# ajyoon/rocoder

Measured on AMD Instinct MI355X. Metric: output Msamples/s, 16384-win f=8 stereo (x CPU-realtime in config), higher is better.
Workload: dtype f32

## Files before the change

rocoder_amd/csrc/rc_hop16k.hip:

```cpp
#include "rc_dit.hpp"

namespace rc {
namespace {

constexpr int f1_idx(int n) { return n + (n >> 5); }
constexpr int HOP2_XBUF = 8192 + 256 + 32;
constexpr int HOP2_LDS_FLOAT2 = HOP2_XBUF + 8 + 32 + 256 + 256 + 16 + 24 + 1024;
constexpr int F3_W[13] = {1, 2, 4, 8, 16, 32, 64, 131, 259, 520, 1038, 2079, 4156};
constexpr int f3_idx(int n) {
    int r = 0;
    for (int i = 0; i < 13; ++i) r += ((n >> i) & 1) * F3_W[i];
    return r;
}

__global__ __launch_bounds__(256, 2) void hop2_kernel(const HopParams p) {
    constexpr int LOG2N = 14, m = 13, M = 1 << m, H = M, T = 256, P = 32, PH = 16;
    constexpr int RES = 512;
    constexpr int SCR = HOP2_XBUF + 8;
    constexpr int T_A = SCR + 32;
    constexpr int T_R = T_A + 256;
    constexpr int T_B = T_R + 256;
    constexpr int T_C = T_B + 16;
    constexpr int T_H = T_C + 24;
    static_assert(T_H + 1024 == HOP2_LDS_FLOAT2, "LDS layout");
// ... 152 lines not shown
            for (int q = 0; q < 16; ++q) {
                const v2f wrv = to_v(wr);
                const v2f wq = q == 0 ? wrv : (q == 8 ? v2f{wr.y, -wr.x}
                               : vcmul(wrv, v2f{W32_RE[q & 15], W32_IM[q & 15]}));
                v2f VA, VB;
                pair_regs_pk<LOG2N>(va[q], vb[15 - q], wq, x0 + (uint32_t)q * dx, key, VA, VB);
                va[q] = VA;
                vb[15 - q] = VB;
            }
        }
        st.mark(10);
        if (tid < 64) {
            const int i = tid;
            if (i <= 16) {
                int ja, ia, ib;
                if (i == 0) { ja = 0; ia = 0; ib = 0; }
                else if (i <= 7) { ja = RES * i; ia = i; ib = 16 - i; }
                else if (i == 8) { ja = RES * 8; ia = 8; ib = 8; }
                else { ja = RES / 2 + RES * (i - 9); ia = 16 + (i - 9); ib = 16 + 15 - (i - 9); }
                const float2 A = lds[SCR + ia], Bp = lds[SCR + ib];
                const float2 w = lds[T_C + (ja >> 8)];
                float2 VA, VB;
                pair_regs<LOG2N>(A, Bp, w, (uint32_t)ja * key.mul + key.k0, key, VA, VB, ja == 0);
                lds[SCR + ia] = VA;
                if (ib != ia) lds[SCR + ib] = VB;
            }
            if (tid == 0) {
#pragma unroll
                for (int q = 0; q < 16; ++q) {
                    va[q] = to_v(lds[SCR + q]);
                    vb[q] = to_v(lds[SCR + 16 + q]);
                }
            }
        }
        st.mark(11);
        v2f pa[16], pb[16];
#pragma unroll
        for (int q = 0; q < 16; ++q) {
            pa[brev_c(q, 4)] = va[q];
            pb[brev_c(q, 4)] = vb[q];
        }
        dit_stages<16, m, 0, 3, 0, true, false>(pa);
        dit_stages<16, m, 0, 3, 0, true, false>(pb);
        st.mark(12);
#pragma unroll
        for (int q = 0; q < 16; ++q) {
            lds[bE3a + f3_idx(q)] = to_f2(pa[q]);
            lds[bE3b + f3_idx(q)] = to_f2(pb[q]);
        }
        st.mark(13);
        __syncthreads();
        st.mark(14);
#pragma unroll
        for (int q = 0; q < P; ++q) v[q] = xld(lds, b4f3 + f3_idx(q << 4));
        dit_stages<32, m, 4, 8, 4, true, true>(v, to_v(lds[T_B + l4]));
        st.mark(15);
#pragma unroll
        for (int q = 0; q < P; ++q) lds[b4f3 + f3_idx(q << 4)] = to_f2(v[q]);
        st.mark(16);
        __syncthreads();
        st.mark(17);
#pragma unroll
        for (int q = 0; q < P; ++q) v[q] = xld(lds, bE4l + f3_idx((q << 8)));
        st.mark(18);
        __syncthreads();
        st.mark(19);
        dit_stages<32, m, 9, 12, 8, true, true>(v, to_v(lds[T_A + tid]));
        st.mark(20);

        epilogue(k, v);
    }
#if RC_STAMP
    if ((tid & 63) == 0 && p.spec) {
        unsigned *dbg = (unsigned *)p.spec + ((size_t)blockIdx.x * (T / 64) + (tid >> 6)) * 32;
        for (int i = 0; i < 32; ++i) dbg[i] = st.acc[i];
    }
#endif
}


constexpr int HOP4_REG = 1040;
constexpr int HOP4_XBUF = 4 * HOP4_REG;
constexpr int HOP4_LDS_FLOAT2 = HOP4_XBUF + 8 + 32 + 256 + 256 + 16 + 24 + 1024;
constexpr int phi_c(int l) { return (l & 1) ? 1 + 2 * (((l >> 1) ^ (l >> 2)) & 1) : 2 * ((l >> 1) & 1); }
constexpr int cidx_c(int l) { return (((l >> 2) & 1) << 1) | ((l >> 3) & 1); }
__device__ __forceinline__ void wave_fence() {
    __builtin_amdgcn_fence(__ATOMIC_RELEASE, "wavefront");
    asm volatile("" ::: "memory");
    __builtin_amdgcn_fence(__ATOMIC_ACQUIRE, "wavefront");
}

#define HOP4_BAR()                                                                    \
    do {                                                                              \
        asm volatile("s_waitcnt lgkmcnt(0)\n\ts_barrier" ::: "memory");                \
    } while (0)
__device__ __forceinline__ float band_gain(const HopParams &p, uint32_t f) {
    return (f - p.band_lo) <= p.band_span ? p.band_gin : p.band_gout;
}
template <int PITCHC, bool BAND = false, bool TABW = false>
__global__ __launch_bounds__(256, 3) void hop4_kernel(const HopParams p) {
    constexpr bool PITCH1 = PITCHC == 1;
    static_assert(!TABW || (PITCH1 && !BAND), "the table-window instantiation exists for pitch 1 without the band mask");
    constexpr int LOG2N = 14, m = 13, M = 1 << m, H = M, T = 256, P = 32, PH = 16;
    constexpr int RES = 512, REG = HOP4_REG;
    constexpr int SCR = HOP4_XBUF + 8;
    constexpr int T_A = SCR + 32;
    constexpr int T_R = T_A + 256;
    constexpr int T_B = T_R + 256;
    constexpr int T_C = T_B + 16;
    constexpr int T_H = T_C + 24;
    static_assert(T_H + 1024 == HOP4_LDS_FLOAT2, "LDS layout");
    extern __shared__ __attribute__((aligned(16))) float2 lds[];
    const int tid = threadIdx.x;
    uint32_t gr = blockIdx.x;
    const bool seam = p.seam_head != nullptr;
    if (seam) {
        unsigned *slot = reinterpret_cast<unsigned *>(lds + SCR);
        if (tid == 0) {
            const uint32_t total = p.runs_per_channel * p.n_channels;
            unsigned got = 0xFFFFFFFFu;
            {
                const uint32_t G = (total + 7u) / 8u;
                unsigned xcc;
                asm volatile("s_getreg_b32 %0, hwreg(HW_REG_XCC_ID)" : "=s"(xcc));
                for (uint32_t i = 0; i < 8u; ++i) {
                    const uint32_t xx = (xcc + i) & 7u, lo = xx * G;
                    if (lo >= total) continue;
                    const uint32_t hi = lo + G < total ? lo + G : total;
                    const uint32_t t = atomicAdd(p.run_counter + xx, 1u);
                    if (t < hi - lo) {
                        got = lo + t;
                        break;
                    }
                }
            }
            *slot = got;
        }
        __syncthreads();
        gr = (uint32_t)__builtin_amdgcn_readfirstlane((int)*reinterpret_cast<volatile unsigned *>(slot));
        __syncthreads();
        if (gr == 0xFFFFFFFFu) return;
    }
    const uint32_t run = gr % p.runs_per_channel;
    const uint32_t ch = gr / p.runs_per_channel;
    const int64_t k_begin = p.hop_first + (int64_t)run * p.run_len;
    int64_t k_end = k_begin + p.run_len;
    if (k_end > p.hop_first + p.hop_count) k_end = p.hop_first + p.hop_count;
    if (k_begin >= k_end) return;
    const bool stash_first = seam && run > 0;
    const bool has_next = seam && run + 1 < p.runs_per_channel;
    GF xc = (GF)p.x + (size_t)ch * p.in_stride;
    GF xt = (GF)p.xtail + (size_t)ch * p.tail_stride;
    GFW outc = (GFW)p.out + (size_t)ch * p.out_stride;
    const unsigned lane2 = 2u * (unsigned)tid;
    GV2 wtab = (GV2)p.wtab;
    const uint32_t pitch = PITCHC ? (uint32_t)PITCHC : p.pitch;

    struct Who {
        int wv, lane, cc, lo4, nib, r, A0;
    };
    int nib_keep, a0_keep;
    {
        const int w_ = tid >> 6, c_ = (tid >> 4) & 3;
        const int nl3 = c_ & 1, nl2 = c_ >> 1, nl0 = w_ & 1;
        const int nl1 = nl0 ? ((w_ >> 1) ^ nl2) : (w_ >> 1);
        nib_keep = (nl3 << 3) | (nl2 << 2) | (nl1 << 1) | nl0;
        a0_keep = w_ * REG + (tid & 63);
    }
    auto who = [&]() {
        int t = tid;
        opaque(t);
        Who w;
        w.wv = t >> 6;
        w.lane = t & 63;
        w.cc = (t >> 4) & 3;
        w.lo4 = t & 15;
        w.nib = nib_keep;
        w.r = (w.lo4 << 4) | w.nib;
        w.A0 = a0_keep;
        return w;
    };
    const int wv = tid >> 6;
    Stamps st;
    st.init();
    v2f tail[PH];
#pragma unroll
    for (int q = 0; q < PH; ++q) tail[q] = v2f{0.f, 0.f};
    {
        lds[T_A + tid] = ldg2(wtab + tid);
        lds[T_R + tid] = ldg2((GV2)p.rtab + tid);
        if (tid < 16) lds[T_B + tid] = ldg2(wtab + 16 * tid);
        if (tid <= 16) lds[T_C + tid] = ldg2(wtab + 128 * tid);
        if (tid == 0) {
            const float2 w256 = ldg2((GV2)p.rtab + 256);
            lds[SCR + 2] = make_float2(-w256.y, w256.x);
        }
        if constexpr (!TABW) {
#pragma unroll
            for (int i = 0; i < 2; ++i) {
                const float2 a = ldg2((GV2)p.hann_rot + 512 * i + 2 * tid);
                const float2 b = ldg2((GV2)p.hann_rot + 512 * i + 2 * tid + 1);
                lds[T_H + 512 * i + 2 * tid] = make_float2(a.x, b.x);
                lds[T_H + 512 * i + 2 * tid + 1] = make_float2(a.y, b.y);
            }
        }
        __syncthreads();
    }
    const v2f half2 = {0.5f, 0.5f};
    auto store_head = [&](int64_t kk, const auto &head) {
        const v2f amp2 = {p.amp, p.amp};
        const v2f cbE = to_v(lds[T_H + 2 * T + 2 * tid]) * amp2, sbE = to_v(lds[T_H + 2 * T + 2 * tid + 1]) * amp2;
        const v2f halfa = half2 * amp2;
        const int64_t g0 = kk * (int64_t)H;
        if constexpr (PITCH1) {
            const unsigned long long da = (unsigned long long)(outc + (g0 - p.out_origin));
            const unsigned dlo = __builtin_amdgcn_readfirstlane((unsigned)da);
            const unsigned dhi = __builtin_amdgcn_readfirstlane((unsigned)(da >> 32));
            GFW dst = (GFW)(((unsigned long long)dhi << 32) | dlo);
            const __amdgpu_buffer_rsrc_t rd = __builtin_amdgcn_make_buffer_rsrc((void *)dst, 0, 0x40000000, 0x00020000);
            typedef unsigned v2u __attribute__((ext_vector_type(2)));
#define HOP4_STORE(o, row)                                                                                                  \
    do {                                                                                                                    \
        if constexpr (!TABW)                                                                             \
            __builtin_amdgcn_raw_buffer_store_b64(v2u{__float_as_uint((o).x), __float_as_uint((o).y)}, rd,                 \
                                                  (int)(4u * lane2), 4 * 2 * T * (row), 2);                                 \
        else __builtin_nontemporal_store(o, (GV2W)(dst + 2 * T * (row) + lane2));                                           \
    } while (0)
            if constexpr (TABW) {
                GF et2 = per_hop(p.env) + lane2;
#pragma unroll
                for (int q0 = 0; q0 < PH; q0 += 4) {
                    float e0[4], e1[4];
#pragma unroll
                    for (int q = 0; q < 4; ++q) {
                        e0[q] = (et2 + 2 * T * (q0 + q))[0];
                        e1[q] = (et2 + 2 * T * (q0 + q))[1];
                    }
#pragma unroll
                    for (int q = 0; q < 4; ++q) {
                        const v2f o = (head[q0 + q] + tail[q0 + q]) * v2f{e0[q], e1[q]} * amp2;
                        HOP4_STORE(o, q0 + q);
                    }
                    __builtin_amdgcn_sched_barrier(0);
                }
                return;
            }
#pragma unroll
            for (int q = 0; q < PH; ++q) {
                const v2f er = __builtin_elementwise_fma(v2f{HANN_E14.s[q], HANN_E14.s[q]}, sbE,
                               __builtin_elementwise_fma(v2f{HANN_E14.c[q], HANN_E14.c[q]}, cbE, halfa));
                const v2f o = (head[q] + tail[q]) * er;
                HOP4_STORE(o, q);
            }
        } else {
            const int64_t kq = g0 / pitch;
            const uint32_t kr = (uint32_t)(g0 % pitch);
            GFW dst = outc + (kq - p.out_origin);
            int t2 = tid;
            opaque(t2);
            const unsigned long long da = (unsigned long long)dst;
            const unsigned dlo = __builtin_amdgcn_readfirstlane((unsigned)da);
            const unsigned dhi = __builtin_amdgcn_readfirstlane((unsigned)(da >> 32));
            const __amdgpu_buffer_rsrc_t rsrc = __builtin_amdgcn_make_buffer_rsrc(
                (void *)(((unsigned long long)dhi << 32) | dlo), 0, 0x40000000, 0x00020000);
            if constexpr (PITCHC > 1) {
                const PitchOffsets<PITCHC> po = pitch_offsets<PITCHC>(kr + 2u * (uint32_t)t2);
#pragma unroll
                for (int q = 0; q < PH; ++q) {
                    const v2f er = __builtin_elementwise_fma(v2f{HANN_E14.s[q], HANN_E14.s[q]}, sbE,
                                   __builtin_elementwise_fma(v2f{HANN_E14.c[q], HANN_E14.c[q]}, cbE, halfa));
                    const v2f o = (head[q] + tail[q]) * er;
                    const float ox = o.x, oy = o.y;
                    pitch_store_pair<PITCHC, 2 * T>(rsrc, po, q, ox, oy);
                }
                return;
            }
            constexpr uint32_t DROP = 0xFFFFFFFCu;
            const uint32_t a00 = kr + 2u * (uint32_t)t2;
            const uint32_t d0 = a00 / pitch;
            uint32_t r = a00 - d0 * pitch, d4 = 4u * d0;
            const uint32_t qs4 = 4u * ((2u * T) / pitch), rs = (2u * T) - (qs4 / 4u) * pitch;
#pragma unroll
            for (int q = 0; q < PH; ++q) {
                const v2f er = __builtin_elementwise_fma(v2f{HANN_E14.s[q], HANN_E14.s[q]}, sbE,
                               __builtin_elementwise_fma(v2f{HANN_E14.c[q], HANN_E14.c[q]}, cbE, halfa));
                const v2f o = (head[q] + tail[q]) * er;
                const float ox = o.x, oy = o.y;
                __builtin_amdgcn_raw_buffer_store_b32(__float_as_int(ox), rsrc, r == 0 ? d4 : DROP, 0, 0);
                __builtin_amdgcn_raw_buffer_store_b32(__float_as_int(oy), rsrc, r + 1 == pitch ? d4 + 4u : DROP, 0, 0);
                d4 += qs4;
                r += rs;
                if (r >= pitch) {
                    r -= pitch;
                    d4 += 4u;
                }
            }
        }
    };
    for (int64_t k = ((k_begin > 0 && !stash_first) ? k_begin - 1 : k_begin); k < k_end; ++k) {
        const PhaseKey key = make_phase_key(p.seed_mixed, p.ch_first + ch, k);
        v2f v[P];
        st.mark(26);
        {
            GF src = hop_src(p, xc, xt, k);
            float xr0[P], xr1[P];
            if constexpr (!TABW) {
                const __amdgpu_buffer_rsrc_t rs = __builtin_amdgcn_make_buffer_rsrc((void *)src, 0, 0x40000000, 0x00020000);
                typedef unsigned v2u __attribute__((ext_vector_type(2)));
#pragma unroll
                for (int q = 0; q < P; ++q) {
                    const v2u x = __builtin_amdgcn_raw_buffer_load_b64(rs, (int)(4u * lane2), 4 * 2 * T * q, 0);
                    xr0[q] = __uint_as_float(x.x);
                    xr1[q] = __uint_as_float(x.y);
                }
            } else {
#pragma unroll
                for (int q = 0; q < P; ++q) {
                    xr0[q] = (src + 2 * T * q)[lane2];
                    xr1[q] = (src + 2 * T * q)[lane2 + 1];
                }
            }
            const v2f cb = to_v(lds[T_H + 2 * tid]), sb = to_v(lds[T_H + 2 * tid + 1]);
            if constexpr (TABW) {
                GF wt2 = per_hop(p.window) + lane2;
#pragma unroll
                for (int q0 = 0; q0 < 16; q0 += 4) {
                    float l0[4], l1[4], h0[4], h1[4];
#pragma unroll
                    for (int q = 0; q < 4; ++q) {
                        l0[q] = (wt2 + 2 * T * (q0 + q))[0];
                        l1[q] = (wt2 + 2 * T * (q0 + q))[1];
                        h0[q] = (wt2 + 2 * T * (q0 + q + 16))[0];
                        h1[q] = (wt2 + 2 * T * (q0 + q + 16))[1];
                    }
#pragma unroll
                    for (int qq = 0; qq < 4; ++qq) {
                        const int q = q0 + qq;
                        const v2f a = v2f{xr0[q], xr1[q]} * v2f{l0[qq], l1[qq]}, xh = v2f{xr0[q + 16], xr1[q + 16]};
                        const v2f wh = v2f{h0[qq], h1[qq]};
                        v[2 * brev_c(q, 4)] = __builtin_elementwise_fma(xh, wh, a);
                        v[2 * brev_c(q, 4) + 1] = __builtin_elementwise_fma(-xh, wh, a);
                    }
                    __builtin_amdgcn_sched_barrier(0);
                }
            } else
#pragma unroll
            for (int q = 0; q < 16; ++q) {
                const v2f wl = __builtin_elementwise_fma(v2f{HANN_W14.s[q], HANN_W14.s[q]}, sb,
                               __builtin_elementwise_fma(v2f{HANN_W14.c[q], HANN_W14.c[q]}, cb, half2));
                const v2f wh = __builtin_elementwise_fma(v2f{HANN_W14.s[q + 16], HANN_W14.s[q + 16]}, sb,
                               __builtin_elementwise_fma(v2f{HANN_W14.c[q + 16], HANN_W14.c[q + 16]}, cb, half2));
                const v2f a = v2f{xr0[q], xr1[q]} * wl, xh = v2f{xr0[q + 16], xr1[q + 16]};
                v[2 * brev_c(q, 4)] = __builtin_elementwise_fma(xh, wh, a);
                v[2 * brev_c(q, 4) + 1] = __builtin_elementwise_fma(-xh, wh, a);
            }
            st.mark(0);
            dit_stages<32, m, 1, 4, 0, false, false>(v);
            st.mark(1);
        }
        wave_fence();
        {
            const Who w = who();
            const int A0 = w.A0, A1 = w.wv * REG + (w.lane ^ 16);
#pragma unroll
            for (int q = 0; q < 16; ++q) lds[((q >> 3) & 1 ? A1 : A0) + q * 64] = to_f2(v[q]);
        }
        st.mark(2);
        HOP4_BAR();
        st.mark(3);
        v2f w2[P];
        {
            const Who w = who();
            const int b4u = (int)(__brev((unsigned)w.lo4) >> 28), l3 = w.nib >> 3;
            const int bE1Ae = w.nib * 64 + b4u + 16 * l3, bE1Ao = w.nib * 64 + b4u - 16 * l3;
#pragma unroll
            for (int j = 0; j < 16; ++j) {
                const int bj = brev_c(j, 4), X = bj & 3;
                w2[2 * j] = to_v(lds[(bj >> 2) * REG + X * 16 + ((X & 1) ? bE1Ao : bE1Ae)]);
            }
        }
        st.mark(4);
        HOP4_BAR();
        st.mark(5);
        {
            int t = tid;
            opaque(t);
            const int bE1Bs = (int)(__brev((unsigned)(t >> 4)) >> 28) * 64 + (int)(__brev((unsigned)(t & 15)) >> 28);
#pragma unroll
            for (int q = 0; q < 16; ++q) lds[phi_c(q) * REG + cidx_c(q) * 16 + bE1Bs] = to_f2(v[16 + q]);
        }
        st.mark(6);
        HOP4_BAR();
        st.mark(7);
        Who w = who();
#pragma unroll
        for (int j = 0; j < 16; ++j) w2[2 * j + 1] = to_v(lds[w.A0 + j * 64]);
        st.mark(8);
        dit_stages<32, m, 5, 8, 4, false, true>(w2, to_v(lds[T_B + w.nib]));
        st.mark(9);
        wave_fence();
        v2f va[16], vb[16];
        {
            w = who();
            const int rlow = (256 - w.r) & 255;
            const int nibb = rlow & 15;
            const int cb = (((nibb >> 2) & 1) << 1) | (nibb >> 3);
            const int bE2A = w.wv * REG + w.lo4 * 65 + w.cc * 16;
            const int bE2B = w.wv * REG + (rlow >> 4) * 65 + cb * 16;
#pragma unroll
            for (int q = 0; q < 16; ++q) lds[w.A0 + q * 65] = to_f2(w2[q]);
            wave_fence();
#pragma unroll
            for (int q = 0; q < 16; ++q) va[q] = to_v(lds[bE2A + q]);
            wave_fence();
#pragma unroll
            for (int q = 0; q < 16; ++q) lds[w.A0 + q * 65] = to_f2(w2[16 + q]);
            wave_fence();
#pragma unroll
            for (int q = 0; q < 16; ++q) vb[q] = to_v(lds[bE2B + q]);
            wave_fence();
        }
        st.mark(10);
        w = who();
        const int r = w.r;
        {
            const v2f wa = to_v(lds[T_A + r]);
            const v2f k16 = {W32_RE[2], W32_IM[2]};
            v2f wb = vcmul(v2f{wa.x, -wa.y}, k16);
            if (tid == 0) wb = v2f{W32_RE[1], W32_IM[1]};
            dit_stages<16, m, 9, 12, 9, false, true>(va, wa);
// ... 27 lines not shown
                               : vcmul(wrv, v2f{W32_RE[q & 15], W32_IM[q & 15]}));
                v2f VA, VB;
                v2f gq = {1.0f, 1.0f};
                if constexpr (BAND) {
                    const uint32_t ja = (uint32_t)r + (uint32_t)RES * (uint32_t)q - ((q >= 8 && is0) ? 3840u : 0u);
                    gq = v2f{band_gain(p, ja), band_gain(p, (uint32_t)M - ja)};
                }
                if (q == 0)
                    pair_regs_pk5<LOG2N, true, BAND>(va[q], vb[15 - q], wq, x0, key, VA, VB, is0, gq);
                else
                    pair_regs_pk5<LOG2N, false, BAND>(va[q], vb[15 - q], wq, (q < 8 ? x0 : x0h) + (uint32_t)q * dx, key, VA, VB,
                                                  false, gq);
                va[q] = VA;
                vb[15 - q] = VB;
            }
        }
        st.mark(12);
        if (wv == 0) {
            v2f V8, V8b;
            const float g8 = BAND ? band_gain(p, 8u * (uint32_t)RES) : 1.0f;
            pair_regs_pk5<LOG2N, false, BAND>(s8, s8, v2f{0.0f, -1.0f}, 8u * (uint32_t)RES * key.mul + key.k0, key, V8, V8b,
                                          false, v2f{g8, g8});
            v2f na[8], nb0[8], nb1[8];
#pragma unroll
            for (int i = 0; i < 8; ++i) {
                na[i] = vsel(is0, i == 0 ? V8 : vb[7 + i], va[8 + i]);
                nb0[i] = vsel(is0, va[8 + i], vb[i]);
                nb1[i] = vsel(is0, vb[i], vb[8 + i]);
            }
#pragma unroll
            for (int i = 0; i < 8; ++i) {
                va[8 + i] = na[i];
                vb[i] = nb0[i];
                vb[8 + i] = nb1[i];
            }
        }
        st.mark(13);
        v2f pa[16], pb[16];
#pragma unroll
        for (int q = 0; q < 16; ++q) {
            pa[brev_c(q, 4)] = va[q];
            pb[brev_c(q, 4)] = vb[q];
        }
        dit_stages<16, m, 0, 3, 0, true, false>(pa);
        dit_stages<16, m, 0, 3, 0, true, false>(pb);
        st.mark(14);
        wave_fence();
        {
            w = who();
            const int bE3A = w.wv * REG + w.lo4 * 65 + w.cc * 16;
            const int nn = (16 - w.nib) & 15;
            const int cs3 = (((nn >> 2) & 1) << 1) | (nn >> 3);
            const int bE3B = w.wv * REG + w.lo4 * 65 + cs3 * 16 + (w.nib == 0 ? 1 : 0);
            const int bE3B0 = bE3B - (w.nib == 0 ? 16 : 0);
#pragma unroll
            for (int q = 0; q < 16; ++q) lds[w.A0 + q * 65] = to_f2(pa[q]);
            wave_fence();
#pragma unroll
            for (int j = 0; j < 16; ++j) v[2 * j] = to_v(lds[bE3A + brev_c(j, 4)]);
            wave_fence();
#pragma unroll
            for (int q = 0; q < 16; ++q) lds[w.A0 + q * 65] = to_f2(pb[q]);
            wave_fence();
#pragma unroll
            for (int j = 0; j < 16; ++j)
                v[2 * j + 1] = to_v(lds[(brev_c(j, 4) == 0 ? bE3B0 : bE3B) + 15 - brev_c(j, 4)]);
            wave_fence();
        }
        st.mark(15);
        w = who();
        dit_stages<32, m, 4, 8, 4, true, true>(v, to_v(lds[T_B + w.lo4]));
        st.mark(16);
        wave_fence();
        {
            w = who();
            const int A0 = w.A0, A1 = w.wv * REG + (w.lane ^ 16);
#pragma unroll
            for (int q = 0; q < 16; ++q) lds[((q & 1) ? A1 : A0) + q * 64] = to_f2(v[q]);
        }
        st.mark(17);
        HOP4_BAR();
        st.mark(18);
        v2f y[P];
        {
            int t = tid;
            opaque(t);
            const int rho8 = t >> 4, l4p = t & 15;
            const int bE4Ae = rho8 * 64 + l4p + 16 * (rho8 & 1), bE4Ao = rho8 * 64 + l4p - 16 * (rho8 & 1);
#pragma unroll
            for (int j = 0; j < 16; ++j) {
                const int nj = brev_c(j, 4), cs = cidx_c(nj);
                y[2 * j] = to_v(lds[phi_c(nj) * REG + 32 * (cs >> 1) + ((cs & 1) ? bE4Ao + 16 : bE4Ae)]);
            }
        }
        st.mark(19);
        HOP4_BAR();
        st.mark(20);
        {
            w = who();
            const int bE4Bs = (int)(__brev((unsigned)w.nib) >> 28) * 64 + w.lo4;
#pragma unroll
            for (int q = 0; q < 16; ++q) lds[(q >> 2) * REG + (q & 3) * 16 + bE4Bs] = to_f2(v[16 + q]);
        }
        st.mark(21);
        HOP4_BAR();
        st.mark(22);
        w = who();
#pragma unroll
        for (int j = 0; j < 16; ++j) y[2 * j + 1] = to_v(lds[w.A0 + j * 64]);
        st.mark(23);
        dit_stages<32, m, 9, 12, 8, true, true>(y, to_v(lds[T_A + tid]));
        st.mark(24);

        const v2f cbW = to_v(lds[T_H + 2 * tid]), sbW = to_v(lds[T_H + 2 * tid + 1]);
        const v2f half2k = {(float)(0.5 * HANN_KAPPA), (float)(0.5 * HANN_KAPPA)};
        if constexpr (TABW) {
            GF wt2 = per_hop(p.window) + lane2;
            const v2f kap = half2k + half2k;
#pragma unroll
            for (int q0 = 0; q0 < P; q0 += 4) {
                float a0[4], a1[4];
#pragma unroll
                for (int q = 0; q < 4; ++q) {
                    a0[q] = (wt2 + 2 * T * (q0 + q))[0];
                    a1[q] = (wt2 + 2 * T * (q0 + q))[1];
                }
#pragma unroll
                for (int q = 0; q < 4; ++q) y[q0 + q] *= v2f{a0[q], a1[q]} * kap;
                __builtin_amdgcn_sched_barrier(0);
            }
        } else
#pragma unroll
        for (int q = 0; q < P; ++q)
            y[q] *= __builtin_elementwise_fma(v2f{HANN_W14K.s[q], HANN_W14K.s[q]}, sbW,
                    __builtin_elementwise_fma(v2f{HANN_W14K.c[q], HANN_W14K.c[q]}, cbW, half2k));
        if (k >= k_begin) {
            if (stash_first && k == k_begin) {
                int t2 = tid;
                opaque(t2);
                unsigned long long *hs = (unsigned long long *)(p.seam_head + (size_t)gr * H) + t2;
#pragma unroll
                for (int q = 0; q < PH; ++q)
                    __hip_atomic_store(hs + T * q, __builtin_bit_cast(unsigned long long, y[q]),
                                       __ATOMIC_RELAXED, __HIP_MEMORY_SCOPE_AGENT);
                asm volatile("s_waitcnt vmcnt(0)" ::: "memory");
                __syncthreads();
                if (tid == 0 && !(p.diag_flags & RC_DIAG_SKIP_SEAM_PUBLISH))
                    __hip_atomic_store(p.seam_flag + gr, p.seam_epoch, __ATOMIC_RELAXED, __HIP_MEMORY_SCOPE_AGENT);
            } else {
                store_head(k, y);
            }
        }
#pragma unroll
        for (int q = 0; q < PH; ++q) tail[q] = y[q + PH];
        st.mark(25);
    }
#if RC_STAMP
    if ((tid & 63) == 0 && p.spec) {
        unsigned *dbg = (unsigned *)p.spec + ((size_t)blockIdx.x * (T / 64) + (tid >> 6)) * 32;
        for (int i = 0; i < 32; ++i) dbg[i] = st.acc[i];
    }
#endif
    if (has_next) {
        unsigned *okw = reinterpret_cast<unsigned *>(lds + SCR);
        if (tid == 0) {
            unsigned ok = 0;
            for (unsigned spin = 0; spin < p.seam_spin_limit; ++spin) {
                if (__hip_atomic_load(p.seam_flag + gr + 1, __ATOMIC_RELAXED, __HIP_MEMORY_SCOPE_AGENT) ==
                    p.seam_epoch) {
                    ok = 1;
                    break;
                }
                __builtin_amdgcn_s_sleep(32);
            }
            if (!ok && p.err_word)
                __hip_atomic_store(p.err_word, RC_ERR_SEAM_TIMEOUT, __ATOMIC_RELAXED, __HIP_MEMORY_SCOPE_SYSTEM);
            *okw = ok;
        }
        __syncthreads();
        if (*reinterpret_cast<volatile unsigned *>(okw) == 0) return;
        const unsigned long long *hs = (const unsigned long long *)(p.seam_head + (size_t)(gr + 1) * H) + tid;
        v2f head[PH];
#pragma unroll
        for (int q = 0; q < PH; ++q)
            head[q] = __builtin_bit_cast(v2f, __hip_atomic_load(hs + T * q, __ATOMIC_RELAXED, __HIP_MEMORY_SCOPE_AGENT));
        store_head(k_end, head);
    }
}

}

hipError_t launch_hop16k(const HopParams &p, hipStream_t s) {
    const dim3 grid(p.runs_per_channel * p.n_channels), block(256);
    const bool hann = p.hann_rot != nullptr;
#if RC_TEST_HOOKS
    if (hann && (p.diag_flags & RC_DIAG_PREV_KERNEL)) return launch_hop16k_prev(p, s);
#endif
    if (hann) {
        const size_t lds4 = sizeof(float2) * (size_t)HOP4_LDS_FLOAT2;
        if (p.band_on) {
            if (p.pitch == 1) hipLaunchKernelGGL((hop4_kernel<1, true>), grid, block, lds4, s, p);
            else hipLaunchKernelGGL((hop4_kernel<0, true>), grid, block, lds4, s, p);
        } else if (p.pitch == 1) hipLaunchKernelGGL((hop4_kernel<1>), grid, block, lds4, s, p);
        else if (p.pitch == 2) hipLaunchKernelGGL((hop4_kernel<2>), grid, block, lds4, s, p);
        else if (p.pitch == 3) hipLaunchKernelGGL((hop4_kernel<3>), grid, block, lds4, s, p);
        else hipLaunchKernelGGL((hop4_kernel<0>), grid, block, lds4, s, p);
    } else {
        if (!p.window || !p.env) return hipErrorInvalidValue;
        if (p.pitch == 1)
            hipLaunchKernelGGL((hop4_kernel<1, false, true>), grid, block, sizeof(float2) * (size_t)HOP4_LDS_FLOAT2, s, p);
        else hipLaunchKernelGGL(hop2_kernel, grid, block, sizeof(float2) * (size_t)HOP2_LDS_FLOAT2, s, p);
    }
    return hipGetLastError();
}
}
```

rocoder_amd/csrc/rc_engine.cpp:

```cpp
#include "../../include/rocoder_hip.h"
#include "rc_kernels.h"
#include "rc_frames.h"
#include "rc_long.h"
#include "rc_rtc.h"
#if defined(RC_HAVE_KERNEL_ID_H)
#include "rc_kernel_id.h"
#else
#define RC_KERNEL_ID "unhashed"
#endif

#include <algorithm>
#include <atomic>
#include <chrono>
#include <cmath>
#include <cstdarg>
#include <cstdint>
#include <cstdio>
#include <cstdlib>
#include <cstring>
#include <deque>
#include <functional>
#include <memory>
#include <new>
#include <string>
// ... 1253 lines not shown
    return (size_t)(offline_windows(p, in_len) * p.window_out_len);
}

uint64_t rc_phase_key(uint64_t seed, uint32_t channel, uint64_t hop) {
    const uint64_t ctr = ((uint64_t)channel << 40) | (hop & 0xFFFFFFFFFFull);
    return mix64(mix64(seed) ^ ctr);
}

uint32_t rc_phase_hash(uint64_t key, uint32_t bin) {
    uint32_t x = bin * ((uint32_t)(key >> 32) | 1u) + (uint32_t)key;
    x ^= x >> 16;
    x *= 0x21F0AAADu;
    x ^= x >> 15;
    x *= 0x735A2D97u;
    x ^= x >> 15;
    return x;
}
float rc_phase_theta(uint64_t key, uint32_t bin, uint32_t n_bins) {
    const uint32_t half = n_bins / 2;
    const bool upper = bin >= half;
    const uint32_t h = rc_phase_hash(key, upper ? bin - half : bin);
    const float u = upper ? (float)(h & 0xFFFFu) * (1.0f / 65536.0f) : (float)(h >> 9) * (1.0f / 8388608.0f);
    return u * 3.14159265358979323846f;
}

int rc_engine_create(const rc_config *cfg, rc_engine **out) try {
    if (!out) return fail(RC_EINVAL, "null out");
    *out = nullptr;
    rc_params par;
    int rc = derive(cfg, &par);
    if (rc) return rc;
    WinPath path;
    int log2n;
    if ((rc = win_path(cfg->window_len, &path, &log2n))) return rc;
    const bool gen = path == WinPath::Gen, lw = path == WinPath::Long, big = path == WinPath::Big;
    int ndev = 0;
    if (hipGetDeviceCount(&ndev) != hipSuccess || ndev <= 0) {
        (void)hipGetLastError();
        return fail(RC_ENODEVICE, "no HIP device available (this library has no CPU fallback)");
    }
    if (cfg->device < 0 || cfg->device >= ndev) return fail(RC_EINVAL, "device %d out of range", cfg->device);
    RC_HIP(hipSetDevice(cfg->device));
    hipDeviceProp_t prop;
    RC_HIP(hipGetDeviceProperties(&prop, cfg->device));
    if (strncmp(prop.gcnArchName, "gfx950", 6) != 0)
        return fail(RC_ENODEVICE, "device %d is %s; this library is built for gfx950 only", cfg->device, prop.gcnArchName);
    rc_engine *e = new (std::nothrow) rc_engine();
    if (!e) return fail(RC_ENOMEM, "out of host memory");
    e->cfg = *cfg;
    e->cfg.window = nullptr;
    e->par = par;
    e->path = path;
    e->log2n = log2n;
    e->device = cfg->device;
    e->n_cu = prop.multiProcessorCount > 0 ? prop.multiProcessorCount : 256;
    e->seed_mixed = mix64(cfg->seed);
    e->ch.resize(cfg->channels);
    e->kernel_next_hop.assign(cfg->channels, 0);
    const uint32_t N = cfg->window_len, M = N / 2, H = N / 2;
    std::vector<float> w(N), env(H);
    if (cfg->window) memcpy(w.data(), cfg->window, N * sizeof(float));
    else hanning(N, w.data());
    crossfade_comp(H, env.data());
    bool default_window = true;
    if (cfg->window) {
        std::vector<float> d(N);
        hanning(N, d.data());
        default_window = memcmp(d.data(), w.data(), N * sizeof(float)) == 0;
    }
    std::vector<float> hann_rot;
    if (default_window && (path == WinPath::Hop || big)) {
        int threads = log2n == 14 ? 256 : 512;
        if (log2n < 14) rc::hop_geometry(log2n, &threads, nullptr);
        hann_rot.resize((size_t)2 * threads * 4);
        for (int part = 0; part < 2; ++part) {
            const double len1 = (double)((part ? H : N) - 1);
            for (int t = 0; t < threads; ++t)
                for (int b = 0; b < 2; ++b) {
                    const double beta = 2.0 * M_PI * (double)(2 * t + b) / len1;
                    hann_rot[((size_t)part * threads + t) * 4 + 2 * b] = (float)cos(beta);
                    hann_rot[((size_t)part * threads + t) * 4 + 2 * b + 1] = (float)sin(beta);
                }
        }
    }
    std::vector<float2> twg;
    if (gen) {
        twg.resize(N);
        for (uint32_t k = 0; k < N; ++k) {
            const double a = -2.0 * M_PI * (double)k / (double)N;
            twg[k] = make_float2((float)cos(a), (float)sin(a));
        }
    }
    std::vector<float2> blt;
    uint32_t bl_log2l = 0;
    if (gen) {
        const uint32_t Mh = N / 2;
        while ((1u << bl_log2l) < 2 * Mh - 1 || bl_log2l < 1) ++bl_log2l;
        const uint32_t L = 1u << bl_log2l;
        blt.resize((size_t)Mh + L / 2 + L);
        std::vector<std::complex<double>> c(Mh), b(L, 0.0), w(L / 2);
        for (uint32_t n = 0; n < Mh; ++n) {
            const uint64_t r = ((uint64_t)n * n) % (2ull * Mh);
            c[n] = std::polar(1.0, -M_PI * (double)r / (double)Mh);
            blt[n] = make_float2((float)c[n].real(), (float)c[n].imag());
            b[n] = std::conj(c[n]);
            if (n) b[L - n] = std::conj(c[n]);
        }
        for (uint32_t k = 0; k < L / 2; ++k) {
            w[k] = std::polar(1.0, -2.0 * M_PI * (double)k / (double)L);
            blt[Mh + k] = make_float2((float)w[k].real(), (float)w[k].imag());
        }
        for (int s = (int)bl_log2l - 1; s >= 0; --s) {
            const uint32_t half = 1u << s;
            for (uint32_t q = 0; q < L / 2; ++q) {
                const uint32_t lo = q & (half - 1), i = ((q >> s) << (s + 1)) | lo, j = i + half;
                const std::complex<double> u = b[i], v = b[j];
                b[i] = u + v;
                b[j] = (u - v) * w[(size_t)lo << (bl_log2l - 1 - s)];
            }
        }
        for (uint32_t i = 0; i < L; ++i)
            blt[(size_t)Mh + L / 2 + i] = make_float2((float)(b[i].real() / L), (float)(b[i].imag() / L));
    }
    std::vector<float2> lwt;
    size_t lw_off[7] = {0, 0, 0, 0, 0, 0, 0};
    uint32_t lw_log2p = 0, lw_log2r = 0, lw_log2c = 0;
    if (lw) {
        const bool pow2 = (N & (N - 1)) == 0;
        if (pow2) {
            while ((1u << lw_log2p) < M) ++lw_log2p;
        } else {
            while ((1ull << lw_log2p) < 2ull * M - 1) ++lw_log2p;
        }
        if (!rc::lw_split(lw_log2p, &lw_log2r, &lw_log2c))
        {
            rc_engine_destroy(e);
            return fail(RC_EUNSUPPORTED, "window_len %u: no four-step split of 2^%u", N, lw_log2p);
        }
        const uint32_t R = 1u << lw_log2r, C = 1u << lw_log2c, P = 1u << lw_log2p, lo_n = 1u << rc::LW_TW_LO_BITS;
        const size_t sizes[7] = {R / 2, C / 2, P >> rc::LW_TW_LO_BITS, lo_n, (size_t)M + 1, pow2 ? 0 : (size_t)M, pow2 ? 0 : (size_t)P};
        size_t total = 0;
        for (int i = 0; i < 7; ++i) {
            lw_off[i] = total;
            total += sizes[i];
        }
        lwt.resize(total);
        auto unit = [](double num, double den) {
            const double a = -2.0 * M_PI * num / den;
            return make_float2((float)cos(a), (float)sin(a));
        };
        for (uint32_t k = 0; k < R / 2; ++k) lwt[lw_off[0] + k] = unit(k, R);
        for (uint32_t k = 0; k < C / 2; ++k) lwt[lw_off[1] + k] = unit(k, C);
        for (size_t k = 0; k < sizes[2]; ++k) lwt[lw_off[2] + k] = unit((double)(k << rc::LW_TW_LO_BITS), P);
        for (uint32_t k = 0; k < lo_n; ++k) lwt[lw_off[3] + k] = unit(k, P);
        for (uint32_t j = 0; j <= M; ++j) lwt[lw_off[4] + j] = unit(j, N);
        if (!pow2) {
            std::vector<double> br((size_t)P, 0.0), bi((size_t)P, 0.0);
            for (uint32_t n = 0; n < M; ++n) {
                const uint64_t r = ((uint64_t)n * n) % (2ull * M);
                const double a = -M_PI * (double)r / (double)M, cr = cos(a), ci = sin(a);
                lwt[lw_off[5] + n] = make_float2((float)cr, (float)ci);
                br[n] = cr;
                bi[n] = -ci;
                if (n) {
                    br[P - n] = cr;
                    bi[P - n] = -ci;
// ... 1813 lines not shown
```

Before: 306,800.

## Interleave final FFT stage and window multiply with output stores in pitch-1 path

For the pitch-1, non-band, analytic-window hop kernel, the last radix-2 DIT stage is split out of dit_stages and run in pairs (i3_pairs), interleaved row by row with windowing, tail hand-over and the output buffer stores. Even rows are stored first, then odd rows, so that store issue overlaps with the remaining butterfly arithmetic instead of waiting for the whole FFT to finish. The input load order is also permuted into bit-reversed order to match. This adds scheduling barriers and more complex control, which may raise register pressure at 3 waves/SIMD occupancy.

```diff
diff --git a/rocoder_amd/csrc/rc_hop16k.hip b/rocoder_amd/csrc/rc_hop16k.hip
--- a/rocoder_amd/csrc/rc_hop16k.hip
+++ b/rocoder_amd/csrc/rc_hop16k.hip
@@ -273,6 +273,27 @@
 __device__ __forceinline__ float band_gain(const HopParams &p, uint32_t f) {
     return (f - p.band_lo) <= p.band_span ? p.band_gin : p.band_gout;
 }
+template <int PAR, int RB, int J0, int NJ>
+__device__ __forceinline__ void i3_pairs(v2f (&y)[32], const v2f base) {
+    constexpr int half = 1 << RB, nc = half / 2;
+#pragma unroll
+    for (int j = J0; j < J0 + NJ; ++j) {
+        const int ia = 4 * j + PAR, ib = 4 * j + 2 + PAR;
+        const int qa = ((ia >> RB) << (RB + 1)) | (ia & (half - 1)), qb = ((ib >> RB) << (RB + 1)) | (ib & (half - 1));
+        const int ca = qa & (half - 1), cb = qb & (half - 1);
+        const int ta = ca < nc ? ca : ca - nc, tb = cb < nc ? cb : cb - nc;
+        const int ka = (ta * (16 >> RB)) & 15, kb = (tb * (16 >> RB)) & 15;
+        const v2f wa = ta == 0 ? base : vcmul(base, v2f{W32_RE[ka], W32_IM[ka]});
+        const v2f wb = tb == 0 ? base : vcmul(base, v2f{W32_RE[kb], W32_IM[kb]});
+        v2f a0 = y[qa], b0 = y[qa | half], a1 = y[qb], b1 = y[qb | half];
+        vdit2_m<true>(a0, b0, wa, ca >= nc, a1, b1, wb, cb >= nc);
+        y[qa] = b0, y[qa | half] = a0, y[qb] = b1, y[qb | half] = a1;
+    }
+}
+template <int V>
+struct IntC {
+    static constexpr int value = V;
+};
 template <int PITCHC, bool BAND = false, bool TABW = false>
 __global__ __launch_bounds__(256, 3) void hop4_kernel(const HopParams p) {
     constexpr bool PITCH1 = PITCHC == 1;
@@ -383,7 +404,9 @@
         __syncthreads();
     }
     const v2f half2 = {0.5f, 0.5f};
-    auto store_head = [&](int64_t kk, const auto &head) {
+    auto store_head = [&](int64_t kk, const auto &head, auto par, auto &&pre) {
+        constexpr int PAR = decltype(par)::value;
+        static_assert(PAR < 0 || (PITCHC != 0 && !TABW), "the runtime-pitch and table-window epilogues walk their rows in order");
         const v2f amp2 = {p.amp, p.amp};
         const v2f cbE = to_v(lds[T_H + 2 * T + 2 * tid]) * amp2, sbE = to_v(lds[T_H + 2 * T + 2 * tid + 1]) * amp2;
         const v2f halfa = half2 * amp2;
@@ -423,10 +446,13 @@
             }
 #pragma unroll
             for (int q = 0; q < PH; ++q) {
+                if (PAR >= 0 && (q & 1) != PAR) continue;
+                pre(q);
                 const v2f er = __builtin_elementwise_fma(v2f{HANN_E14.s[q], HANN_E14.s[q]}, sbE,
                                __builtin_elementwise_fma(v2f{HANN_E14.c[q], HANN_E14.c[q]}, cbE, halfa));
                 const v2f o = (head[q] + tail[q]) * er;
                 HOP4_STORE(o, q);
+                if (PAR >= 0) __builtin_amdgcn_sched_barrier(0);
             }
         } else {
             const int64_t kq = g0 / pitch;
@@ -443,11 +469,14 @@
                 const PitchOffsets<PITCHC> po = pitch_offsets<PITCHC>(kr + 2u * (uint32_t)t2);
 #pragma unroll
                 for (int q = 0; q < PH; ++q) {
+                    if (PAR >= 0 && (q & 1) != PAR) continue;
+                    pre(q);
                     const v2f er = __builtin_elementwise_fma(v2f{HANN_E14.s[q], HANN_E14.s[q]}, sbE,
                                    __builtin_elementwise_fma(v2f{HANN_E14.c[q], HANN_E14.c[q]}, cbE, halfa));
                     const v2f o = (head[q] + tail[q]) * er;
                     const float ox = o.x, oy = o.y;
                     pitch_store_pair<PITCHC, 2 * T>(rsrc, po, q, ox, oy);
+                    if (PAR >= 0) __builtin_amdgcn_sched_barrier(0);
                 }
                 return;
             }
@@ -480,18 +509,21 @@
         {
             GF src = hop_src(p, xc, xt, k);
             float xr0[P], xr1[P];
+            auto LQ = [](int j) { return PITCH1 ? brev_c(j, 4) : j; };
             if constexpr (!TABW) {
                 const __amdgpu_buffer_rsrc_t rs = __builtin_amdgcn_make_buffer_rsrc((void *)src, 0, 0x40000000, 0x00020000);
                 typedef unsigned v2u __attribute__((ext_vector_type(2)));
 #pragma unroll
-                for (int q = 0; q < P; ++q) {
+                for (int j = 0; j < P; ++j) {
+                    const int q = PITCH1 ? LQ(j >> 1) + 16 * (j & 1) : j;
                     const v2u x = __builtin_amdgcn_raw_buffer_load_b64(rs, (int)(4u * lane2), 4 * 2 * T * q, 0);
                     xr0[q] = __uint_as_float(x.x);
                     xr1[q] = __uint_as_float(x.y);
                 }
             } else {
 #pragma unroll
-                for (int q = 0; q < P; ++q) {
+                for (int j = 0; j < P; ++j) {
+                    const int q = PITCH1 ? LQ(j >> 1) + 16 * (j & 1) : j;
                     xr0[q] = (src + 2 * T * q)[lane2];
                     xr1[q] = (src + 2 * T * q)[lane2 + 1];
                 }
@@ -503,15 +535,16 @@
                 for (int q0 = 0; q0 < 16; q0 += 4) {
                     float l0[4], l1[4], h0[4], h1[4];
 #pragma unroll
-                    for (int q = 0; q < 4; ++q) {
-                        l0[q] = (wt2 + 2 * T * (q0 + q))[0];
-                        l1[q] = (wt2 + 2 * T * (q0 + q))[1];
-                        h0[q] = (wt2 + 2 * T * (q0 + q + 16))[0];
-                        h1[q] = (wt2 + 2 * T * (q0 + q + 16))[1];
+                    for (int qq = 0; qq < 4; ++qq) {
+                        const int q = LQ(q0 + qq);
+                        l0[qq] = (wt2 + 2 * T * q)[0];
+                        l1[qq] = (wt2 + 2 * T * q)[1];
+                        h0[qq] = (wt2 + 2 * T * (q + 16))[0];
+                        h1[qq] = (wt2 + 2 * T * (q + 16))[1];
                     }
 #pragma unroll
                     for (int qq = 0; qq < 4; ++qq) {
-                        const int q = q0 + qq;
+                        const int q = LQ(q0 + qq);
                         const v2f a = v2f{xr0[q], xr1[q]} * v2f{l0[qq], l1[qq]}, xh = v2f{xr0[q + 16], xr1[q + 16]};
                         const v2f wh = v2f{h0[qq], h1[qq]};
                         v[2 * brev_c(q, 4)] = __builtin_elementwise_fma(xh, wh, a);
@@ -521,7 +554,8 @@
                 }
             } else
 #pragma unroll
-            for (int q = 0; q < 16; ++q) {
+            for (int j = 0; j < 16; ++j) {
+                const int q = LQ(j);
                 const v2f wl = __builtin_elementwise_fma(v2f{HANN_W14.s[q], HANN_W14.s[q]}, sb,
                                __builtin_elementwise_fma(v2f{HANN_W14.c[q], HANN_W14.c[q]}, cb, half2));
                 const v2f wh = __builtin_elementwise_fma(v2f{HANN_W14.s[q + 16], HANN_W14.s[q + 16]}, sb,
@@ -742,50 +776,95 @@
 #pragma unroll
         for (int j = 0; j < 16; ++j) y[2 * j + 1] = to_v(lds[w.A0 + j * 64]);
         st.mark(23);
-        dit_stages<32, m, 9, 12, 8, true, true>(y, to_v(lds[T_A + tid]));
-        st.mark(24);
-
+        constexpr bool DRIP = PITCH1 && !BAND && !TABW;
         const v2f cbW = to_v(lds[T_H + 2 * tid]), sbW = to_v(lds[T_H + 2 * tid + 1]);
         const v2f half2k = {(float)(0.5 * HANN_KAPPA), (float)(0.5 * HANN_KAPPA)};
-        if constexpr (TABW) {
-            GF wt2 = per_hop(p.window) + lane2;
-            const v2f kap = half2k + half2k;
-#pragma unroll
-            for (int q0 = 0; q0 < P; q0 += 4) {
-                float a0[4], a1[4];
-#pragma unroll
-                for (int q = 0; q < 4; ++q) {
-                    a0[q] = (wt2 + 2 * T * (q0 + q))[0];
-                    a1[q] = (wt2 + 2 * T * (q0 + q))[1];
-                }
-#pragma unroll
-                for (int q = 0; q < 4; ++q) y[q0 + q] *= v2f{a0[q], a1[q]} * kap;
-                __builtin_amdgcn_sched_barrier(0);
-            }
-        } else
-#pragma unroll
-        for (int q = 0; q < P; ++q)
-            y[q] *= __builtin_elementwise_fma(v2f{HANN_W14K.s[q], HANN_W14K.s[q]}, sbW,
-                    __builtin_elementwise_fma(v2f{HANN_W14K.c[q], HANN_W14K.c[q]}, cbW, half2k));
-        if (k >= k_begin) {
-            if (stash_first && k == k_begin) {
-                int t2 = tid;
-                opaque(t2);
-                unsigned long long *hs = (unsigned long long *)(p.seam_head + (size_t)gr * H) + t2;
-#pragma unroll
-                for (int q = 0; q < PH; ++q)
-                    __hip_atomic_store(hs + T * q, __builtin_bit_cast(unsigned long long, y[q]),
-                                       __ATOMIC_RELAXED, __HIP_MEMORY_SCOPE_AGENT);
-                asm volatile("s_waitcnt vmcnt(0)" ::: "memory");
-                __syncthreads();
-                if (tid == 0 && !(p.diag_flags & RC_DIAG_SKIP_SEAM_PUBLISH))
-                    __hip_atomic_store(p.seam_flag + gr, p.seam_epoch, __ATOMIC_RELAXED, __HIP_MEMORY_SCOPE_AGENT);
+        auto winmul = [&](int q) {
+            v2f yw = y[q] * __builtin_elementwise_fma(v2f{HANN_W14K.s[q], HANN_W14K.s[q]}, sbW,
+                            __builtin_elementwise_fma(v2f{HANN_W14K.c[q], HANN_W14K.c[q]}, cbW, half2k));
+            asm("" : "+v"(yw));
+            y[q] = yw;
+        };
+        const bool stash = stash_first && k == k_begin;
+        bool dripped = false;
+        if constexpr (!DRIP) {
+            dit_stages<32, m, 9, 12, 8, true, true>(y, to_v(lds[T_A + tid]));
+            st.mark(24);
+        } else {
+            const v2f w12 = to_v(lds[T_A + tid]);
+            dit_stages<32, m, 9, 11, 8, true, true>(y, vcsq(w12));
+            i3_pairs<0, 4, 0, 4>(y, w12);
+            st.mark(24);
+            auto hand_over = [&](int q) {
+                winmul(q + PH);
+                tail[q] = y[q + PH];
+            };
+            if (k >= k_begin && !stash) {
+                dripped = true;
+                store_head(k, y, IntC<0>{}, [&](int q) {
+                    switch (q >> 1) {
+                    case 0: i3_pairs<1, 4, 0, 1>(y, w12); break;
+                    case 2: i3_pairs<1, 4, 1, 1>(y, w12); break;
+                    case 4: i3_pairs<1, 4, 2, 1>(y, w12); break;
+                    case 6: i3_pairs<1, 4, 3, 1>(y, w12); break;
+                    default:
+                        if (q >= 4) hand_over(q - 4);
+                        hand_over(q - 2);
+                        break;
+                    }
+                    winmul(q);
+                });
+                store_head(k, y, IntC<1>{}, [&](int q) {
+                    hand_over(q == 1 ? PH - 2 : q - 2);
+                    winmul(q);
+                });
+                hand_over(PH - 1);
             } else {
-                store_head(k, y);
-            }
-        }
-#pragma unroll
-        for (int q = 0; q < PH; ++q) tail[q] = y[q + PH];
+                i3_pairs<1, 4, 0, 4>(y, w12);
+            }
+        }
+        if (!dripped) {
+            if constexpr (TABW) {
+                GF wt2 = per_hop(p.window) + lane2;
+                const v2f kap = half2k + half2k;
+#pragma unroll
+                for (int q0 = 0; q0 < P; q0 += 4) {
+                    float a0[4], a1[4];
+#pragma unroll
+                    for (int q = 0; q < 4; ++q) {
+                        a0[q] = (wt2 + 2 * T * (q0 + q))[0];
+                        a1[q] = (wt2 + 2 * T * (q0 + q))[1];
+                    }
+#pragma unroll
+                    for (int q = 0; q < 4; ++q) y[q0 + q] *= v2f{a0[q], a1[q]} * kap;
+                    __builtin_amdgcn_sched_barrier(0);
+                }
+            } else
+#pragma unroll
+            for (int q = 0; q < P; ++q) winmul(q);
+            if (k >= k_begin) {
+                if (stash) {
+                    int t2 = tid;
+                    opaque(t2);
+                    unsigned long long *hs = (unsigned long long *)(p.seam_head + (size_t)gr * H) + t2;
+#pragma unroll
+                    for (int q = 0; q < PH; ++q)
+                        __hip_atomic_store(hs + T * q, __builtin_bit_cast(unsigned long long, y[q]),
+                                           __ATOMIC_RELAXED, __HIP_MEMORY_SCOPE_AGENT);
+                    asm volatile("s_waitcnt vmcnt(0)" ::: "memory");
+                    __syncthreads();
+                    if (tid == 0 && !(p.diag_flags & RC_DIAG_SKIP_SEAM_PUBLISH)) {
+                        unsigned epoch = p.seam_epoch;
+                        asm volatile("" : "+s"(epoch));
+                        __hip_atomic_store(p.seam_flag + gr, epoch, __ATOMIC_RELAXED, __HIP_MEMORY_SCOPE_AGENT);
+                    }
+                } else if constexpr (!DRIP) {
+                    store_head(k, y, IntC<-1>{}, [](int) {});
+                }
+            }
+#pragma unroll
+            for (int q = 0; q < PH; ++q) tail[q] = y[q + PH];
+        }
         st.mark(25);
     }
 #if RC_STAMP
@@ -817,7 +896,7 @@
 #pragma unroll
         for (int q = 0; q < PH; ++q)
             head[q] = __builtin_bit_cast(v2f, __hip_atomic_load(hs + T * q, __ATOMIC_RELAXED, __HIP_MEMORY_SCOPE_AGENT));
-        store_head(k_end, head);
+        store_head(k_end, head, IntC<-1>{}, [](int) {});
     }
 }
 
```

Measured after the change: 305,900. No clear change (-0.3%).

## Add wide-store hop4 variant with 16-byte LDS reads and b128 output stores

Applied to the files above, without the earlier changes.

Adds a WIDE instantiation of the 16k hop kernel for pitch 1. Each thread now owns four adjacent samples, so it can read LDS with 16-byte vector loads, run a reworked final DIT stage set (dit_i3_wide) using paired twiddles, and write output with 128-bit buffer stores instead of 64-bit ones. To support this, extra Hann rotation tables are precomputed on the host and the LDS layout gains 768 float2 of space. The variant is used only when the output pointer, origin and stride are 16-byte aligned. The added LDS and register pressure could lower occupancy below the declared three blocks per CU.

```diff
diff --git a/rocoder_amd/csrc/rc_engine.cpp b/rocoder_amd/csrc/rc_engine.cpp
--- a/rocoder_amd/csrc/rc_engine.cpp
+++ b/rocoder_amd/csrc/rc_engine.cpp
@@ -1359,6 +1359,18 @@
                     hann_rot[((size_t)part * threads + t) * 4 + 2 * b + 1] = (float)sin(beta);
                 }
         }
+        if (log2n == 14) {
+            hann_rot.resize((size_t)4 * threads * 4);
+            for (int part = 0; part < 2; ++part) {
+                const double len1 = (double)((part ? H : N) - 1);
+                for (int u = 0; u < threads; ++u)
+                    for (int b = 0; b < 2; ++b) {
+                        const double beta = 2.0 * M_PI * (double)(4 * u + b) / len1;
+                        hann_rot[((size_t)(2 + part) * threads + u) * 4 + 2 * b] = (float)cos(beta);
+                        hann_rot[((size_t)(2 + part) * threads + u) * 4 + 2 * b + 1] = (float)sin(beta);
+                    }
+            }
+        }
     }
     std::vector<float2> twg;
     if (gen) {
diff --git a/rocoder_amd/csrc/rc_hop16k.hip b/rocoder_amd/csrc/rc_hop16k.hip
--- a/rocoder_amd/csrc/rc_hop16k.hip
+++ b/rocoder_amd/csrc/rc_hop16k.hip
@@ -258,6 +258,7 @@
 constexpr int HOP4_REG = 1040;
 constexpr int HOP4_XBUF = 4 * HOP4_REG;
 constexpr int HOP4_LDS_FLOAT2 = HOP4_XBUF + 8 + 32 + 256 + 256 + 16 + 24 + 1024;
+constexpr int HOP4_WIDE_EXTRA = 256 + 512;
 constexpr int phi_c(int l) { return (l & 1) ? 1 + 2 * (((l >> 1) ^ (l >> 2)) & 1) : 2 * ((l >> 1) & 1); }
 constexpr int cidx_c(int l) { return (((l >> 2) & 1) << 1) | ((l >> 3) & 1); }
 __device__ __forceinline__ void wave_fence() {
@@ -273,19 +274,71 @@
 __device__ __forceinline__ float band_gain(const HopParams &p, uint32_t f) {
     return (f - p.band_lo) <= p.band_span ? p.band_gin : p.band_gout;
 }
-template <int PITCHC, bool BAND = false, bool TABW = false>
+constexpr uint32_t RC_DIAG_HOP4_NARROW = 16;
+
+__device__ __forceinline__ void dit_i3_wide(v2f (&v)[32], v2f w0, v2f w1) {
+    v2f bases[2][4];
+    bases[0][3] = w0;
+    bases[1][3] = w1;
+#pragma unroll
+    for (int k = 2; k >= 0; --k) {
+        bases[0][k] = vcsq(bases[0][k + 1]);
+        bases[1][k] = vcsq(bases[1][k + 1]);
+    }
+#pragma unroll
+    for (int k = 0; k < 4; ++k) {
+        const int half = 1 << k;
+        const int nc = half > 1 ? half / 2 : 1;
+        v2f tw[2][4];
+#pragma unroll
+        for (int c = 0; c < 4; ++c) {
+            if (c >= nc) continue;
+            const int kidx = c * (16 >> k);
+            const v2f kc = {W32_RE[kidx & 15], W32_IM[kidx & 15]};
+            tw[0][c] = c == 0 ? bases[0][k] : vcmul(bases[0][k], kc);
+            tw[1][c] = c == 0 ? bases[1][k] : vcmul(bases[1][k], kc);
+        }
+#pragma unroll
+        for (int i = 0; i < 8; ++i) {
+            const int c0 = ((i >> k) << (k + 1)) | (i & (half - 1)), c1 = c0 | half;
+            const int cc = c0 & (half - 1);
+            const bool rot = cc >= nc;
+            const int ti = rot ? cc - nc : cc;
+            v2f a0 = v[2 * c0], b0 = v[2 * c1], a1 = v[2 * c0 + 1], b1 = v[2 * c1 + 1];
+            vdit2_m<true>(a0, b0, tw[0][ti], rot, a1, b1, tw[1][ti], rot);
+            v[2 * c0] = b0, v[2 * c1] = a0, v[2 * c0 + 1] = b1, v[2 * c1 + 1] = a1;
+        }
+    }
+}
+
+constexpr HannK make_hann_k_wide(double amp, int len, int count) {
+    HannK k{};
+    for (int q = 0; q < 32; ++q) {
+        const double a = q < count ? 2.0 * CX_PI * (1024.0 * (q >> 1) + 2.0 * (q & 1)) / (double)(len - 1) : 0.0;
+        k.c[q] = (float)(-amp * cx_cos(a));
+        k.s[q] = (float)(amp * cx_sin(a));
+    }
+    return k;
+}
+__device__ constexpr HannK HANN_E14W = make_hann_k_wide(HANN_ENV_AMP, 8192, 16);
+__device__ constexpr HannK HANN_W14KW = make_hann_k_wide(0.5 * HANN_KAPPA, 16384, 32);
+
+template <int PITCHC, bool BAND = false, bool TABW = false, bool WIDE = false>
 __global__ __launch_bounds__(256, 3) void hop4_kernel(const HopParams p) {
     constexpr bool PITCH1 = PITCHC == 1;
     static_assert(!TABW || (PITCH1 && !BAND), "the table-window instantiation exists for pitch 1 without the band mask");
+    static_assert(!WIDE || (PITCH1 && !TABW), "the wide-store instantiations exist for pitch 1 with the computed window");
     constexpr int LOG2N = 14, m = 13, M = 1 << m, H = M, T = 256, P = 32, PH = 16;
     constexpr int RES = 512, REG = HOP4_REG;
     constexpr int SCR = HOP4_XBUF + 8;
     constexpr int T_A = SCR + 32;
-    constexpr int T_R = T_A + 256;
+    constexpr int T_R = T_A + (WIDE ? 512 : 256);
     constexpr int T_B = T_R + 256;
     constexpr int T_C = T_B + 16;
     constexpr int T_H = T_C + 24;
-    static_assert(T_H + 1024 == HOP4_LDS_FLOAT2, "LDS layout");
+    static_assert(T_H + (WIDE ? 1536 : 1024) == HOP4_LDS_FLOAT2 + (WIDE ? HOP4_WIDE_EXTRA : 0), "LDS layout");
+    static_assert(T_A % 2 == 0 && T_H % 2 == 0 && REG % 2 == 0, "16-byte LDS reads");
+    typedef float v4f __attribute__((ext_vector_type(4), may_alias));
     extern __shared__ __attribute__((aligned(16))) float2 lds[];
     const int tid = threadIdx.x;
     uint32_t gr = blockIdx.x;
@@ -357,6 +410,11 @@
         return w;
     };
     const int wv = tid >> 6;
+    auto wide_u = [&]() {
+        int t = tid;
+        opaque(t);
+        return (t & 31) | ((t >> 6) << 5) | (((t >> 5) & 1) << 7);
+    };
     Stamps st;
     st.init();
     v2f tail[PH];
@@ -373,19 +431,22 @@
         }
         if constexpr (!TABW) {
 #pragma unroll
-            for (int i = 0; i < 2; ++i) {
-                const float2 a = ldg2((GV2)p.hann_rot + 512 * i + 2 * tid);
-                const float2 b = ldg2((GV2)p.hann_rot + 512 * i + 2 * tid + 1);
+            for (int i = 0; i < (WIDE ? 3 : 2); ++i) {
+                const int part = WIDE && i ? i + 1 : i;
+                const float2 a = ldg2((GV2)p.hann_rot + 512 * part + 2 * tid);
+                const float2 b = ldg2((GV2)p.hann_rot + 512 * part + 2 * tid + 1);
                 lds[T_H + 512 * i + 2 * tid] = make_float2(a.x, b.x);
                 lds[T_H + 512 * i + 2 * tid + 1] = make_float2(a.y, b.y);
             }
+            if constexpr (WIDE) lds[T_A + 256 + tid] = ldg2(wtab + 256 + tid);
         }
         __syncthreads();
     }
     const v2f half2 = {0.5f, 0.5f};
     auto store_head = [&](int64_t kk, const auto &head) {
         const v2f amp2 = {p.amp, p.amp};
-        const v2f cbE = to_v(lds[T_H + 2 * T + 2 * tid]) * amp2, sbE = to_v(lds[T_H + 2 * T + 2 * tid + 1]) * amp2;
+        const int hrot = WIDE ? 4 * T + 2 * wide_u() : 2 * T + 2 * tid;
+        const v2f cbE = to_v(lds[T_H + hrot]) * amp2, sbE = to_v(lds[T_H + hrot + 1]) * amp2;
         const v2f halfa = half2 * amp2;
         const int64_t g0 = kk * (int64_t)H;
         if constexpr (PITCH1) {
@@ -421,6 +482,25 @@
                 }
                 return;
             }
+            if constexpr (WIDE) {
+                typedef unsigned v4u __attribute__((ext_vector_type(4)));
+                const int lane16 = 16 * wide_u();
+#pragma unroll
+                for (int c = 0; c < PH / 2; ++c) {
+                    v2f o[2];
+#pragma unroll
+                    for (int b0 = 0; b0 < 2; ++b0) {
+                        const int q = 2 * c + b0;
+                        const v2f er = __builtin_elementwise_fma(v2f{HANN_E14W.s[q], HANN_E14W.s[q]}, sbE,
+                                       __builtin_elementwise_fma(v2f{HANN_E14W.c[q], HANN_E14W.c[q]}, cbE, halfa));
+                        o[b0] = (head[q] + tail[q]) * er;
+                    }
+                    __builtin_amdgcn_raw_buffer_store_b128(v4u{__float_as_uint(o[0].x), __float_as_uint(o[0].y),
+                                                               __float_as_uint(o[1].x), __float_as_uint(o[1].y)},
+                                                           rd, lane16, 4 * 1024 * c, 2);
+                }
+                return;
+            }
 #pragma unroll
             for (int q = 0; q < PH; ++q) {
                 const v2f er = __builtin_elementwise_fma(v2f{HANN_E14.s[q], HANN_E14.s[q]}, sbE,
@@ -715,7 +795,21 @@
         HOP4_BAR();
         st.mark(18);
         v2f y[P];
-        {
+        if constexpr (WIDE) {
+            int t = tid;
+            opaque(t);
+            const int lane = t & 63;
+            const int rho = ((lane >> 3) & 3) | ((t >> 6) << 2);
+            const int bE4Ae = rho * 64 + 2 * (lane & 7) + 16 * (rho & 1), bE4Ao = rho * 64 + 2 * (lane & 7) - 16 * (rho & 1);
+#pragma unroll
+            for (int c = 0; c < 16; ++c) {
+                const int nj = brev_c(c, 4), cs = cidx_c(nj);
+                const v4f g = *reinterpret_cast<const v4f *>(
+                    lds + (phi_c(nj) * REG + 32 * (cs >> 1) + ((cs & 1) ? bE4Ao + 16 : bE4Ae)));
+                y[2 * c] = v2f{g.x, g.y};
+                y[2 * c + 1] = v2f{g.z, g.w};
+            }
+        } else {
             int t = tid;
             opaque(t);
             const int rho8 = t >> 4, l4p = t & 15;
@@ -739,13 +833,28 @@
         HOP4_BAR();
         st.mark(22);
         w = who();
+        if constexpr (WIDE) {
+            if (w.lane & 32) {
+                const int bE4Bl = w.wv * REG + 2 * (w.lane & 31);
+#pragma unroll
+                for (int c = 0; c < 16; ++c) {
+                    const v4f g = *reinterpret_cast<const v4f *>(lds + (bE4Bl + c * 64));
+                    y[2 * c] = v2f{g.x, g.y};
+                    y[2 * c + 1] = v2f{g.z, g.w};
+                }
+            }
+        } else
 #pragma unroll
         for (int j = 0; j < 16; ++j) y[2 * j + 1] = to_v(lds[w.A0 + j * 64]);
         st.mark(23);
-        dit_stages<32, m, 9, 12, 8, true, true>(y, to_v(lds[T_A + tid]));
+        if constexpr (WIDE) {
+            const v4f wab = *reinterpret_cast<const v4f *>(lds + (T_A + 2 * wide_u()));
+            dit_i3_wide(y, v2f{wab.x, wab.y}, v2f{wab.z, wab.w});
+        } else dit_stages<32, m, 9, 12, 8, true, true>(y, to_v(lds[T_A + tid]));
         st.mark(24);
 
-        const v2f cbW = to_v(lds[T_H + 2 * tid]), sbW = to_v(lds[T_H + 2 * tid + 1]);
+        const int wrot = WIDE ? 2 * T + 2 * wide_u() : 2 * tid;
+        const v2f cbW = to_v(lds[T_H + wrot]), sbW = to_v(lds[T_H + wrot + 1]);
         const v2f half2k = {(float)(0.5 * HANN_KAPPA), (float)(0.5 * HANN_KAPPA)};
         if constexpr (TABW) {
             GF wt2 = per_hop(p.window) + lane2;
@@ -764,9 +873,11 @@
             }
         } else
 #pragma unroll
-        for (int q = 0; q < P; ++q)
-            y[q] *= __builtin_elementwise_fma(v2f{HANN_W14K.s[q], HANN_W14K.s[q]}, sbW,
-                    __builtin_elementwise_fma(v2f{HANN_W14K.c[q], HANN_W14K.c[q]}, cbW, half2k));
+        for (int q = 0; q < P; ++q) {
+            constexpr const HannK &HK = WIDE ? HANN_W14KW : HANN_W14K;
+            y[q] *= __builtin_elementwise_fma(v2f{HK.s[q], HK.s[q]}, sbW,
+                    __builtin_elementwise_fma(v2f{HK.c[q], HK.c[q]}, cbW, half2k));
+        }
         if (k >= k_begin) {
             if (stash_first && k == k_begin) {
                 int t2 = tid;
@@ -831,10 +942,18 @@
 #endif
     if (hann) {
         const size_t lds4 = sizeof(float2) * (size_t)HOP4_LDS_FLOAT2;
+        const size_t lds4w = sizeof(float2) * (size_t)(HOP4_LDS_FLOAT2 + HOP4_WIDE_EXTRA);
+        bool wide = p.pitch == 1 && !(p.diag_flags & RC_DIAG_HOP4_NARROW);
+        if (wide) {
+            const int64_t base = (int64_t)((uintptr_t)p.out >> 2) - p.out_origin;
+            wide = ((uintptr_t)p.out & 3) == 0 && (base & 3) == 0 && (p.n_channels <= 1 || (p.out_stride & 3) == 0);
+        }
         if (p.band_on) {
-            if (p.pitch == 1) hipLaunchKernelGGL((hop4_kernel<1, true>), grid, block, lds4, s, p);
+            if (wide) hipLaunchKernelGGL((hop4_kernel<1, true, false, true>), grid, block, lds4w, s, p);
+            else if (p.pitch == 1) hipLaunchKernelGGL((hop4_kernel<1, true>), grid, block, lds4, s, p);
             else hipLaunchKernelGGL((hop4_kernel<0, true>), grid, block, lds4, s, p);
-        } else if (p.pitch == 1) hipLaunchKernelGGL((hop4_kernel<1>), grid, block, lds4, s, p);
+        } else if (wide) hipLaunchKernelGGL((hop4_kernel<1, false, false, true>), grid, block, lds4w, s, p);
+        else if (p.pitch == 1) hipLaunchKernelGGL((hop4_kernel<1>), grid, block, lds4, s, p);
         else if (p.pitch == 2) hipLaunchKernelGGL((hop4_kernel<2>), grid, block, lds4, s, p);
         else if (p.pitch == 3) hipLaunchKernelGGL((hop4_kernel<3>), grid, block, lds4, s, p);
         else hipLaunchKernelGGL((hop4_kernel<0>), grid, block, lds4, s, p);
```

Result: no change. 307,000 before, 307,600 after, median of 3 (+0.2%).
